# RomanJuranek/librectify

Hardware: AMD Instinct MI355X
Metric: Mpix/s end-to-end (detect+VP) on 4K frames, batch call of 64 frames, 5 in flight (higher is better)
Workload: dtype f32

## Files before the change

librectify_amd/csrc/kernels_fit.hip:

```cpp
#include <algorithm>
#include <cstring>

#include <atomic>

#include "common.h"

namespace lramd {
namespace {

constexpr uint32_t kNoComp = 0xFFFFFFFFu;

constexpr uint32_t kSortLds = 1024;
constexpr uint32_t kSortLdsBig = 16384;
constexpr uint32_t kHugeShift = 14;
constexpr uint32_t kHugeFlag = 0x80000000u;
constexpr int kOffPer = 8;
constexpr uint32_t kOffChunk = 256 * kOffPer;

__device__ __forceinline__ void chunk_counts(const int32_t* __restrict__ seed_size, uint32_t n_seeds, int min_size, int fit_min,
                                             uint32_t k0, int (&sz)[kOffPer], uint32_t& c, uint32_t& p, uint32_t& rc, uint32_t& rp) {
    c = p = rc = rp = 0;
#pragma unroll
    for (int j = 0; j < kOffPer; ++j) {
        sz[j] = (k0 + j < n_seeds) ? seed_size[k0 + j] : 0;
        if (sz[j] > min_size) {
            rc += 1u;
            rp += (uint32_t)sz[j];
        }
        if (sz[j] > fit_min) {
            c += 1u;
            p += (uint32_t)sz[j];
        }
    }
}

__global__ __launch_bounds__(256) void component_offsets_kernel(const int32_t* __restrict__ seed_size,
                                                                const uint32_t* __restrict__ n_ptr, uint32_t cap,
                                                                int min_size, int fit_min, unsigned long long* __restrict__ status, uint32_t tag,
                                                                uint32_t* __restrict__ comp_rank,
                                                                uint32_t* __restrict__ comp_seed,
                                                                uint32_t* __restrict__ comp_off,
                                                                uint32_t* __restrict__ totals, uint32_t* __restrict__ fit_totals,
                                                                uint32_t* __restrict__ large_list,
                                                                uint32_t large_cap, uint32_t* __restrict__ n_large,
                                                                uint32_t* __restrict__ cursor, uint32_t* __restrict__ huge_list,
                                                                uint32_t huge_max) {
    __shared__ uint32_t s_c[4], s_p[4], s_cc[4], s_cp[4], s_rc[4], s_rp[4];
    const uint32_t n_seeds = min(*n_ptr, cap);
    const int tid = threadIdx.x, lane = tid & 63, wv = tid >> 6;
    const uint32_t k0 = blockIdx.x * kOffChunk + (uint32_t)tid * kOffPer;
    int sz[kOffPer];
    uint32_t c, p, rc, rp;
    chunk_counts(seed_size, n_seeds, min_size, fit_min, k0, sz, c, p, rc, rp);
    uint32_t ic = c, ip = p;
#pragma unroll
    for (int off = 1; off < 64; off <<= 1) {
        const uint32_t tc = (uint32_t)__shfl_up((int)ic, off);
        const uint32_t tp = (uint32_t)__shfl_up((int)ip, off);
        if (lane >= off) {
            ic += tc;
            ip += tp;
        }
    }
#pragma unroll
    for (int off = 32; off >= 1; off >>= 1) {
        rc += (uint32_t)__shfl_xor((int)rc, off);
        rp += (uint32_t)__shfl_xor((int)rp, off);
    }
    if (lane == 63) {
        s_c[wv] = ic;
        s_p[wv] = ip;
        s_rc[wv] = rc;
        s_rp[wv] = rp;
    }
    __syncthreads();
    if (tid == 0) {
        const unsigned long long t = (unsigned long long)tag << 32;
        const unsigned long long wc = t | (unsigned long long)(s_c[0] + s_c[1] + s_c[2] + s_c[3]);
        const unsigned long long wp = t | (unsigned long long)(s_p[0] + s_p[1] + s_p[2] + s_p[3]);
        if (blockIdx.x == 0) {
#pragma unroll
            for (int i = 0; i < 4; ++i) __hip_atomic_store(&n_large[i], 0u, __ATOMIC_RELAXED, __HIP_MEMORY_SCOPE_AGENT);
            __hip_atomic_store(&totals[0], 0u, __ATOMIC_RELAXED, __HIP_MEMORY_SCOPE_AGENT);
            __hip_atomic_store(&totals[1], 0u, __ATOMIC_RELAXED, __HIP_MEMORY_SCOPE_AGENT);
            __hip_atomic_store(&status[0], wc, __ATOMIC_RELEASE, __HIP_MEMORY_SCOPE_AGENT);
            __hip_atomic_store(&status[1], wp, __ATOMIC_RELEASE, __HIP_MEMORY_SCOPE_AGENT);
        } else {
            __hip_atomic_store(&status[2u * blockIdx.x], wc, __ATOMIC_RELAXED, __HIP_MEMORY_SCOPE_AGENT);
            __hip_atomic_store(&status[2u * blockIdx.x + 1u], wp, __ATOMIC_RELAXED, __HIP_MEMORY_SCOPE_AGENT);
        }
    }
    uint32_t cc = 0, cp = 0;
    for (uint32_t i = (uint32_t)tid; i < blockIdx.x; i += 256) {
        unsigned long long wc = 0ull, wp = 0ull;
        for (uint32_t spins = 0; spins < (1u << 22); ++spins) {
            wc = __hip_atomic_load(&status[2u * i], __ATOMIC_RELAXED, __HIP_MEMORY_SCOPE_AGENT);
            wp = __hip_atomic_load(&status[2u * i + 1u], __ATOMIC_RELAXED, __HIP_MEMORY_SCOPE_AGENT);
            if ((uint32_t)(wc >> 32) == tag && (uint32_t)(wp >> 32) == tag) break;
            __builtin_amdgcn_s_sleep(2);
        }
        cc += (uint32_t)wc;
        cp += (uint32_t)wp;
    }
#pragma unroll
    for (int off = 32; off >= 1; off >>= 1) {
        cc += (uint32_t)__shfl_xor((int)cc, off);
        cp += (uint32_t)__shfl_xor((int)cp, off);
    }
    if (lane == 0) {
        s_cc[wv] = cc;
        s_cp[wv] = cp;
    }
    __syncthreads();
    if (tid == 0) {
        const uint32_t wrc = s_rc[0] + s_rc[1] + s_rc[2] + s_rc[3], wrp = s_rp[0] + s_rp[1] + s_rp[2] + s_rp[3];
        if (wrc != 0u) {
            __hip_atomic_fetch_add(&totals[0], wrc, __ATOMIC_RELAXED, __HIP_MEMORY_SCOPE_AGENT);
            __hip_atomic_fetch_add(&totals[1], wrp, __ATOMIC_RELAXED, __HIP_MEMORY_SCOPE_AGENT);
        }
    }
    uint32_t rank = s_cc[0] + s_cc[1] + s_cc[2] + s_cc[3] + ic - c;
    uint32_t off_px = s_cp[0] + s_cp[1] + s_cp[2] + s_cp[3] + ip - p;
    for (int i = 0; i < wv; ++i) {
        rank += s_c[i];
        off_px += s_p[i];
    }
#pragma unroll
    for (int j = 0; j < kOffPer; ++j) {
        const uint32_t k = k0 + j;
        if (k < n_seeds) {
            const bool keep = sz[j] > fit_min;
            comp_rank[k] = keep ? rank : kNoComp;
            if (keep) {
                comp_seed[rank] = k;
                comp_off[rank] = off_px;
                if (sz[j] > (int)kSortLds) large_list[large_cap - 1u - atomicAdd(n_large + 1, 1u)] = rank;
                else if (sz[j] > 64) large_list[atomicAdd(n_large, 1u)] = rank;
                uint32_t cur = 0u;
                if (sz[j] > (int)kSortLdsBig && huge_max != 0u) {
                    const uint32_t hi = atomicAdd(n_large + 2, 1u);
                    if (hi < huge_max) {
                        cur = hi | kHugeFlag;
                        huge_list[hi] = rank;
                    }
                }
                cursor[rank] = cur;
                rank += 1u;
                off_px += (uint32_t)sz[j];
            }
        }
    }
    if (blockIdx.x == gridDim.x - 1 && tid == 255) {
        fit_totals[0] = rank;
        fit_totals[1] = off_px;
        comp_off[rank] = off_px;
    }
}

__global__ __launch_bounds__(256) void component_scatter_kernel(const uint32_t* __restrict__ label, size_t npix,
                                                                const uint32_t* __restrict__ comp_rank,
                                                                const uint32_t* __restrict__ comp_off,
                                                                uint32_t* __restrict__ cursor,
                                                                uint32_t* __restrict__ px, uint32_t* __restrict__ huge_tab,
                                                                uint32_t nb) {
    const int lane = threadIdx.x & 63;
    const size_t step = (size_t)gridDim.x * 256;
    const size_t n_pad = (npix + 255) / 256 * 256;
    constexpr int kU = 4;
    for (size_t i0 = (size_t)blockIdx.x * 256 + threadIdx.x; i0 < n_pad; i0 += step * kU) {
        uint32_t l[kU], r[kU];
#pragma unroll
        for (int u = 0; u < kU; ++u) {
            const size_t i = i0 + step * (size_t)u;
            l[u] = i < npix ? label[i] : kLabelFree;
        }
#pragma unroll
        for (int u = 0; u < kU; ++u) r[u] = l[u] != kLabelFree ? comp_rank[l[u]] : kNoComp;
#pragma unroll
        for (int u = 0; u < kU; ++u) {
            const size_t i = i0 + step * (size_t)u;
            if (i >= n_pad) break;
            uint64_t todo = __ballot(r[u] != kNoComp);
            while (todo != 0ull) {
                const int leader = __builtin_ctzll(todo);
                const uint32_t rl = (uint32_t)__builtin_amdgcn_readlane((int)r[u], leader);
                const uint64_t same = __ballot(r[u] == rl) & todo;
                uint32_t base = 0;
                if (lane == leader) {
                    const uint32_t o0 = comp_off[rl], o1 = comp_off[rl + 1u];
                    uint32_t hi = 0u;
                    if (o1 - o0 > kSortLdsBig) hi = cursor[rl];
                    if (hi & kHugeFlag) base = atomicAdd(&huge_tab[(size_t)(hi & ~kHugeFlag) * nb + (uint32_t)(i >> kHugeShift)], (uint32_t)__popcll(same));
                    else base = o0 + atomicAdd(&cursor[rl], (uint32_t)__popcll(same));
                }
                base = (uint32_t)__builtin_amdgcn_readlane((int)base, leader);
                if ((same >> lane) & 1ull) px[base + (uint32_t)__popcll(same & ((1ull << lane) - 1ull))] = (uint32_t)i;
                todo &= ~same;
            }
        }
    }
}

__device__ inline float wave_tree(float v) {
#pragma unroll
    for (int off = 32; off >= 1; off >>= 1) v = v + __shfl_xor(v, off);
    return v;
}

__device__ inline void major_axis_2x2(float a_, float b_, float c_, float& d_r, float& d_c) {
    const double a = a_, b = b_, c = c_;
    const double hd = (a - c) * 0.5;
    const double rad = sqrt(hd * hd + b * b);
    const double lmax = (a + c) * 0.5 + rad;
    double vr, vc;
    if (a >= c) {
        vr = lmax - c;
        vc = b;
    } else {
        vr = b;
        vc = lmax - a;
    }
    const double nn = sqrt(vr * vr + vc * vc);
    if (nn > 0.0) {
        vr = vr / nn;
        vc = vc / nn;
    } else {
        vr = 1.0;
        vc = 0.0;
    }
    float fr = (float)vr, fc = (float)vc;
    if (fr < fc || (fr == fc && fr < 0.0f)) {
        fr = -fr;
        fc = -fc;
    }
    d_r = fr;
    d_c = fc;
}

template <int kThreads, class Keys>
__device__ __forceinline__ void bitonic_sort(Keys& key, uint32_t P) {
    for (uint32_t k = 2; k <= P; k <<= 1)
        for (uint32_t j = k >> 1; j > 0; j >>= 1) {
            for (uint32_t t = threadIdx.x; t < P / 2; t += kThreads) {
                const uint32_t i = 2 * t - (t & (j - 1));
                const uint32_t a = key[i], b = key[i + j];
                const bool up = (i & k) == 0;
                if ((a > b) == up) {
                    key[i] = b;
                    key[i + j] = a;
                }
            }
            __syncthreads();
        }
}

__global__ __launch_bounds__(256) void component_sort_large_kernel(const uint32_t* __restrict__ px_in,
                                                                   uint32_t* __restrict__ px_out,
                                                                   const uint32_t* __restrict__ comp_off,
                                                                   const uint32_t* __restrict__ large_list,
                                                                   const uint32_t* __restrict__ n_large) {
    __shared__ uint32_t s_key[kSortLds];
    const uint32_t n_list = n_large[0];
    for (uint32_t li = blockIdx.x; li < n_list; li += gridDim.x) {
        const uint32_t comp = large_list[li];
        const uint32_t off = comp_off[comp];
        const uint32_t n = comp_off[comp + 1] - off;
        uint32_t P = 128;
        while (P < n) P <<= 1;
        for (uint32_t i = threadIdx.x; i < P; i += 256) s_key[i] = i < n ? px_in[off + i] : 0xFFFFFFFFu;
        __syncthreads();
        bitonic_sort<256>(s_key, P);
        for (uint32_t i = threadIdx.x; i < n; i += 256) px_out[off + i] = s_key[i];
        __syncthreads();
    }
}

template <bool kGlobal>
__global__ __launch_bounds__(1024) void component_sort_big_kernel(const uint32_t* __restrict__ px_in,
                                                                  uint32_t* __restrict__ px_out,
                                                                  const uint32_t* __restrict__ comp_off,
                                                                  const uint32_t* __restrict__ large_list,
                                                                  uint32_t large_cap,
                                                                  const uint32_t* __restrict__ n_large,
                                                                  uint32_t* __restrict__ scratch,
                                                                  const uint32_t* __restrict__ cursor) {
    __shared__ uint32_t s_key[kGlobal ? 1 : kSortLdsBig];
    const uint32_t n_list = n_large[1];
    for (uint32_t li = blockIdx.x; li < n_list; li += gridDim.x) {
        const uint32_t comp = large_list[large_cap - 1u - li];
        const uint32_t off = comp_off[comp];
        const uint32_t n = comp_off[comp + 1] - off;
        if ((n > kSortLdsBig) != kGlobal) continue;
        if (kGlobal && cursor != nullptr && (cursor[comp] & kHugeFlag)) continue;
        uint32_t P = 2048;
        while (P < n) P <<= 1;
        if (!kGlobal) {
            for (uint32_t i = threadIdx.x; i < P; i += 1024) s_key[i] = i < n ? px_in[off + i] : 0xFFFFFFFFu;
            __syncthreads();
            bitonic_sort<1024>(s_key, P);
            for (uint32_t i = threadIdx.x; i < n; i += 1024) px_out[off + i] = s_key[i];
            __syncthreads();
        } else {
            for (uint32_t i = threadIdx.x; i < P; i += 1024) scratch[i] = i < n ? px_in[off + i] : 0xFFFFFFFFu;
            __syncthreads();
            bitonic_sort<1024>(scratch, P);
            for (uint32_t i = threadIdx.x; i < n; i += 1024) px_out[off + i] = scratch[i];
            __syncthreads();
        }
    }
}

__global__ __launch_bounds__(256) void huge_count_kernel(const uint32_t* __restrict__ label, size_t npix,
                                                         const uint32_t* __restrict__ comp_rank,
                                                         const uint32_t* __restrict__ comp_off,
                                                         const uint32_t* __restrict__ cursor, uint32_t* __restrict__ huge_tab,
                                                         uint32_t nb, const uint32_t* __restrict__ huge_list, uint32_t huge_max,
                                                         uint4* __restrict__ jobs, uint32_t* __restrict__ n_large) {
    const uint32_t n_huge = min(n_large[2], huge_max);
    if (n_huge == 0u) return;
    const int lane = threadIdx.x & 63;
    const size_t step = (size_t)gridDim.x * 256;
    const size_t n_pad = (npix + 255) / 256 * 256;
    for (size_t i = (size_t)blockIdx.x * 256 + threadIdx.x; i < n_pad; i += step) {
        const uint32_t l = i < npix ? label[i] : kLabelFree;
        const uint32_t r = l != kLabelFree ? comp_rank[l] : kNoComp;
        uint32_t hi = 0u;
        if (r != kNoComp && comp_off[r + 1u] - comp_off[r] > kSortLdsBig) hi = cursor[r];
        uint64_t todo = __ballot((hi & kHugeFlag) != 0u);
        while (todo != 0ull) {
            const int leader = __builtin_ctzll(todo);
            const uint32_t hl = (uint32_t)__builtin_amdgcn_readlane((int)hi, leader);
            const uint64_t same = __ballot(hi == hl) & todo;
            if (lane == leader) atomicAdd(&huge_tab[(size_t)(hl & ~kHugeFlag) * nb + (uint32_t)(i >> kHugeShift)], (uint32_t)__popcll(same));
            todo &= ~same;
        }
    }
    __shared__ uint32_t s_last;
    __syncthreads();
    if (threadIdx.x == 0) {
        __threadfence();
        s_last = atomicAdd(n_large + 6, 1u) == gridDim.x - 1u ? 1u : 0u;
    }
    __syncthreads();
    if (s_last == 0u) return;
    __threadfence();
    if (threadIdx.x == 0) n_large[6] = 0u;
    for (uint32_t h = threadIdx.x >> 6; h < n_huge; h += 4u) {
        const uint32_t rank = huge_list[h];
        uint32_t run = comp_off[rank];
        for (uint32_t b0 = 0; b0 < nb; b0 += 64u) {
            const uint32_t b = b0 + (uint32_t)lane;
            uint32_t* e = &huge_tab[(size_t)h * nb + b];
            const uint32_t cnt = b < nb ? __hip_atomic_load(e, __ATOMIC_RELAXED, __HIP_MEMORY_SCOPE_AGENT) : 0u;
            uint32_t inc = cnt;
#pragma unroll
            for (int off = 1; off < 64; off <<= 1) {
                const uint32_t t = (uint32_t)__shfl_up((int)inc, off);
                if (lane >= off) inc += t;
            }
            const uint32_t start = run + inc - cnt;
            if (cnt != 0u) {
                *e = start;
                jobs[atomicAdd(n_large + 3, 1u)] = make_uint4(start, cnt, h * nb + b, 0u);
            }
            run += (uint32_t)__shfl((int)inc, 63);
        }
    }
}

__global__ __launch_bounds__(1024) void huge_sort_kernel(const uint32_t* __restrict__ px_in, uint32_t* __restrict__ px_out,
                                                         const uint4* __restrict__ jobs, uint32_t* __restrict__ huge_tab,
                                                         const uint32_t* __restrict__ n_large) {
    __shared__ uint32_t s_key[kSortLdsBig];
    const uint32_t n_jobs = n_large[3];
    for (uint32_t j = blockIdx.x; j < n_jobs; j += gridDim.x) {
        const uint4 job = jobs[j];
        const uint32_t off = job.x, n = job.y;
        uint32_t P = 64;
        while (P < n) P <<= 1;
        for (uint32_t i = threadIdx.x; i < P; i += 1024) s_key[i] = i < n ? px_in[off + i] : 0xFFFFFFFFu;
        __syncthreads();
        bitonic_sort<1024>(s_key, P);
        for (uint32_t i = threadIdx.x; i < n; i += 1024) px_out[off + i] = s_key[i];
        if (threadIdx.x == 0) huge_tab[job.z] = 0u;
        __syncthreads();
    }
}

template <int kU>
__device__ __forceinline__ void fit_large(const uint32_t* __restrict__ px, uint32_t comp, uint32_t off, uint32_t n, float s, float c,
                                          uint32_t uw, const float* __restrict__ dx, const float* __restrict__ dy,
                                          float* __restrict__ scratch_w, LineSegment* __restrict__ out, int lane) {
    float acc = 0.f;
    for (uint32_t i0 = lane; i0 < n; i0 += 64u * kU) {
        uint32_t p[kU];
        float gx[kU], gy[kU];
#pragma unroll
        for (int u = 0; u < kU; ++u) {
            const uint32_t i = i0 + 64u * (uint32_t)u;
            p[u] = i < n ? px[off + i] : 0u;
        }
#pragma unroll
        for (int u = 0; u < kU; ++u) {
            gx[u] = dx[p[u]];
            gy[u] = dy[p[u]];
        }
#pragma unroll
        for (int u = 0; u < kU; ++u) {
            const uint32_t i = i0 + 64u * (uint32_t)u;
            if (i < n) {
                const float wv = directional(gx[u], gy[u], s, c);
                scratch_w[off + i] = wv;
                acc = acc + wv;
            }
        }
    }
    const float S = wave_tree(acc);

    float ar = 0.f, ac = 0.f;
    for (uint32_t i0 = lane; i0 < n; i0 += 64u * kU) {
        uint32_t p[kU];
        float wq[kU];
#pragma unroll
        for (int u = 0; u < kU; ++u) {
            const uint32_t i = i0 + 64u * (uint32_t)u;
            p[u] = i < n ? px[off + i] : 0u;
            wq[u] = i < n ? scratch_w[off + i] : 0.f;
        }
#pragma unroll
        for (int u = 0; u < kU; ++u) {
            const uint32_t i = i0 + 64u * (uint32_t)u;
            if (i < n) {
                const float r = (float)(p[u] / uw), cc = (float)(p[u] % uw);
                const float wn = wq[u] / S;
                ar = ar + wn * r;
                ac = ac + wn * cc;
            }
        }
    }
    const float a_r = wave_tree(ar), a_c = wave_tree(ac);

    float crr = 0.f, crc = 0.f, ccc = 0.f;
    for (uint32_t i0 = lane; i0 < n; i0 += 64u * kU) {
        uint32_t p[kU];
        float wq[kU];
#pragma unroll
        for (int u = 0; u < kU; ++u) {
            const uint32_t i = i0 + 64u * (uint32_t)u;
            p[u] = i < n ? px[off + i] : 0u;
            wq[u] = i < n ? scratch_w[off + i] : 0.f;
        }
#pragma unroll
        for (int u = 0; u < kU; ++u) {
            const uint32_t i = i0 + 64u * (uint32_t)u;
            if (i < n) {
                const float cr = (float)(p[u] / uw) - a_r, cc = (float)(p[u] % uw) - a_c;
                const float wn = wq[u] / S;
                const float t = cr * wn, u2 = cc * wn;
                crr = crr + t * cr;
                crc = crc + t * cc;
                ccc = ccc + u2 * cc;
            }
        }
    }
    const float cov_rr = wave_tree(crr), cov_rc = wave_tree(crc), cov_cc = wave_tree(ccc);

    float d_r, d_c;
    major_axis_2x2(cov_rr, cov_rc, cov_cc, d_r, d_c);
    const float n_r = -d_c, n_c = d_r;

    float t0 = INFINITY, t1 = -INFINITY, es = 0.f;
    for (uint32_t i0 = lane; i0 < n; i0 += 64u * kU) {
        uint32_t p[kU];
#pragma unroll
        for (int u = 0; u < kU; ++u) {
            const uint32_t i = i0 + 64u * (uint32_t)u;
            p[u] = i < n ? px[off + i] : 0u;
        }
#pragma unroll
        for (int u = 0; u < kU; ++u) {
            const uint32_t i = i0 + 64u * (uint32_t)u;
            if (i < n) {
                const float cr = (float)(p[u] / uw) - a_r, cc = (float)(p[u] % uw) - a_c;
                const float t = cr * d_r + cc * d_c;
                t0 = fminf(t0, t);
                t1 = fmaxf(t1, t);
                es = es + fabsf(cr * n_r + cc * n_c);
            }
        }
    }
#pragma unroll
    for (int o = 32; o >= 1; o >>= 1) {
        t0 = fminf(t0, __shfl_xor(t0, o));
        t1 = fmaxf(t1, __shfl_xor(t1, o));
    }
    const float esum = wave_tree(es);
    if (lane == 0) {
        LineSegment l;
        l.x1 = a_c + d_c * t0;
        l.y1 = a_r + d_r * t0;
        l.x2 = a_c + d_c * t1;
        l.y2 = a_r + d_r * t1;
        l.weight = S / (float)n;
        l.err = esum / (float)n;
        l.group_id = -1;
        out[comp] = l;
    }
}

__global__ __launch_bounds__(256) void fit_kernel(const uint32_t* __restrict__ px, const uint32_t* __restrict__ px_unsorted,
                                                  const uint32_t* __restrict__ comp_off,
                                                  const uint32_t* __restrict__ comp_seed, const uint32_t* __restrict__ n_comp_ptr,
                                                  const int32_t* __restrict__ seed_bin, const float* __restrict__ dx,
                                                  const float* __restrict__ dy, int w, BinTrig trig,
                                                  float* __restrict__ scratch_w, LineSegment* __restrict__ out,
                                                  const uint32_t* __restrict__ huge_cursor) {
    const int lane = threadIdx.x & 63;
    const uint32_t comp = blockIdx.x * 4 + (threadIdx.x >> 6);
    if (comp >= *n_comp_ptr) return;
    const uint32_t off = comp_off[comp];
    const uint32_t n = comp_off[comp + 1] - off;
    const int b = seed_bin[comp_seed[comp]];
    const float s = trig.st[b], c = trig.ct[b];
    const uint32_t uw = (uint32_t)w;

    if (n <= 64u) {
        const bool has = (uint32_t)lane < n;
        const uint32_t key = has ? px_unsorted[off + lane] : 0xFFFFFFFFu;
        uint32_t rank = 0;
#pragma unroll
        for (int j = 0; j < 64; ++j) rank += ((uint32_t)__builtin_amdgcn_readlane((int)key, j) < key) ? 1u : 0u;
        const uint32_t p_sorted = (uint32_t)__builtin_amdgcn_ds_permute((int)(min(rank, 63u) << 2), (int)key);
        const uint32_t p = has ? p_sorted : 0u;
        float wv = 0.f;
        if (has) wv = directional(dx[p], dy[p], s, c);
        float acc = 0.f;
        if (has) acc = acc + wv;
        const float S = wave_tree(acc);
        const float r = (float)(p / uw), cq = (float)(p % uw);
        const float wn = wv / S;
        float ar = 0.f, ac = 0.f;
        if (has) {
            ar = ar + wn * r;
            ac = ac + wn * cq;
        }
        const float a_r = wave_tree(ar), a_c = wave_tree(ac);
        const float cr = r - a_r, cc = cq - a_c;
        float crr = 0.f, crc = 0.f, ccc = 0.f;
        if (has) {
            const float t = cr * wn, u = cc * wn;
            crr = crr + t * cr;
            crc = crc + t * cc;
            ccc = ccc + u * cc;
        }
        const float cov_rr = wave_tree(crr), cov_rc = wave_tree(crc), cov_cc = wave_tree(ccc);
        float d_r, d_c;
        major_axis_2x2(cov_rr, cov_rc, cov_cc, d_r, d_c);
        const float n_r = -d_c, n_c = d_r;
        float t0 = INFINITY, t1 = -INFINITY, es = 0.f;
        if (has) {
            const float t = cr * d_r + cc * d_c;
            t0 = fminf(t0, t);
            t1 = fmaxf(t1, t);
            es = es + fabsf(cr * n_r + cc * n_c);
        }
#pragma unroll
        for (int o = 32; o >= 1; o >>= 1) {
            t0 = fminf(t0, __shfl_xor(t0, o));
            t1 = fmaxf(t1, __shfl_xor(t1, o));
        }
        const float esum = wave_tree(es);
        if (lane == 0) {
            LineSegment l;
            l.x1 = a_c + d_c * t0;
            l.y1 = a_r + d_r * t0;
            l.x2 = a_c + d_c * t1;
            l.y2 = a_r + d_r * t1;
            l.weight = S / (float)n;
            l.err = esum / (float)n;
            l.group_id = -1;
            out[comp] = l;
        }
        return;
    }

    if (huge_cursor != nullptr && n > kSortLdsBig && (huge_cursor[comp] & kHugeFlag) != 0u) return;
    fit_large<8>(px, comp, off, n, s, c, uw, dx, dy, scratch_w, out, lane);
}

__device__ __forceinline__ float huge_chunk_sum(float acc, const float* __restrict__ v, uint32_t cn, int lane) {
    for (uint32_t j0 = (uint32_t)lane; j0 < cn; j0 += 64u * 16u) {
        float t[16];
#pragma unroll
        for (int u = 0; u < 16; ++u) {
            const uint32_t j = j0 + 64u * (uint32_t)u;
            t[u] = j < cn ? v[j] : 0.f;
        }
#pragma unroll
        for (int u = 0; u < 16; ++u)
            if (j0 + 64u * (uint32_t)u < cn) acc = acc + t[u];
    }
    return acc;
}
constexpr int kHugeTerms = 24576;
constexpr size_t kHugeLdsBytes = (size_t)kHugeTerms * sizeof(float);
__global__ __launch_bounds__(1024) void fit_huge_kernel(const uint32_t* __restrict__ px, const uint32_t* __restrict__ comp_off,
                                                        const uint32_t* __restrict__ comp_seed, const uint32_t* __restrict__ huge_list,
                                                        const uint32_t* __restrict__ n_large, uint32_t huge_max,
                                                        const int32_t* __restrict__ seed_bin, const float* __restrict__ dx,
                                                        const float* __restrict__ dy, int w, BinTrig trig,
                                                        float* __restrict__ scratch_w, LineSegment* __restrict__ out) {
    extern __shared__ float s_terms[];
    __shared__ float s_res[3];
    __shared__ float s_mm[2][16];
    if (blockIdx.x >= min(n_large[2], huge_max)) return;
    const uint32_t comp = huge_list[blockIdx.x];
    const uint32_t off = comp_off[comp];
    const uint32_t n = comp_off[comp + 1] - off;
    const int b = seed_bin[comp_seed[comp]];
    const float s = trig.st[b], c = trig.ct[b];
    const uint32_t uw = (uint32_t)w;
    const int tid = (int)threadIdx.x, lane = tid & 63, wave = tid >> 6;

    float acc = 0.f;
    {
        constexpr uint32_t kC = 16384u;
        constexpr int kE = (int)(kC / 1024u);
        for (uint32_t c0 = 0; c0 < n; c0 += kC) {
            const uint32_t cn = min(kC, n - c0);
            uint32_t p[kE];
            float gx[kE], gy[kE];
#pragma unroll
            for (int e = 0; e < kE; ++e) {
                const uint32_t j = (uint32_t)tid + 1024u * (uint32_t)e;
                p[e] = j < cn ? px[off + c0 + j] : 0u;
            }
#pragma unroll
            for (int e = 0; e < kE; ++e) {
                gx[e] = dx[p[e]];
                gy[e] = dy[p[e]];
            }
#pragma unroll
            for (int e = 0; e < kE; ++e) {
                const uint32_t j = (uint32_t)tid + 1024u * (uint32_t)e;
                if (j < cn) {
                    const float wv = directional(gx[e], gy[e], s, c);
                    scratch_w[off + c0 + j] = wv;
                    s_terms[j] = wv;
                }
            }
            __syncthreads();
            if (wave == 0) acc = huge_chunk_sum(acc, s_terms, cn, lane);
            __syncthreads();
        }
    }
    if (wave == 0) {
        const float t = wave_tree(acc);
        if (lane == 0) s_res[0] = t;
    }
    __syncthreads();
    const float S = s_res[0];
    __syncthreads();

    acc = 0.f;
    {
        constexpr uint32_t kC = kHugeTerms / 2;
        constexpr int kE = (int)(kC / 1024u);
        for (uint32_t c0 = 0; c0 < n; c0 += kC) {
            const uint32_t cn = min(kC, n - c0);
            uint32_t q[kE];
            float wq[kE];
#pragma unroll
            for (int e = 0; e < kE; ++e) {
                const uint32_t j = (uint32_t)tid + 1024u * (uint32_t)e;
                q[e] = j < cn ? px[off + c0 + j] : 0u;
                wq[e] = j < cn ? scratch_w[off + c0 + j] : 0.f;
            }
#pragma unroll
            for (int e = 0; e < kE; ++e) {
                const uint32_t j = (uint32_t)tid + 1024u * (uint32_t)e;
                if (j < cn) {
                    const float r = (float)(q[e] / uw), cc = (float)(q[e] % uw);
                    const float wn = wq[e] / S;
                    s_terms[j] = wn * r;
                    s_terms[kC + j] = wn * cc;
                }
            }
            __syncthreads();
            if (wave < 2) acc = huge_chunk_sum(acc, s_terms + (size_t)wave * kC, cn, lane);
            __syncthreads();
        }
    }
    if (wave < 2) {
        const float t = wave_tree(acc);
        if (lane == 0) s_res[wave] = t;
    }
    __syncthreads();
    const float a_r = s_res[0], a_c = s_res[1];
    __syncthreads();

    acc = 0.f;
    {
        constexpr uint32_t kC = kHugeTerms / 3;
        constexpr int kE = (int)(kC / 1024u);
        static_assert(kC % 1024u == 0u, "a chunk is a whole number of elements per thread");
        for (uint32_t c0 = 0; c0 < n; c0 += kC) {
            const uint32_t cn = min(kC, n - c0);
            uint32_t q[kE];
            float wq[kE];
#pragma unroll
            for (int e = 0; e < kE; ++e) {
                const uint32_t j = (uint32_t)tid + 1024u * (uint32_t)e;
                q[e] = j < cn ? px[off + c0 + j] : 0u;
                wq[e] = j < cn ? scratch_w[off + c0 + j] : 0.f;
            }
#pragma unroll
            for (int e = 0; e < kE; ++e) {
                const uint32_t j = (uint32_t)tid + 1024u * (uint32_t)e;
                if (j < cn) {
                    const float cr = (float)(q[e] / uw) - a_r, cc = (float)(q[e] % uw) - a_c;
                    const float wn = wq[e] / S;
                    const float t = cr * wn, u2 = cc * wn;
                    s_terms[j] = t * cr;
                    s_terms[kC + j] = t * cc;
                    s_terms[2u * kC + j] = u2 * cc;
                }
            }
            __syncthreads();
            if (wave < 3) acc = huge_chunk_sum(acc, s_terms + (size_t)wave * kC, cn, lane);
            __syncthreads();
        }
    }
    if (wave < 3) {
        const float t = wave_tree(acc);
        if (lane == 0) s_res[wave] = t;
    }
    __syncthreads();
    const float cov_rr = s_res[0], cov_rc = s_res[1], cov_cc = s_res[2];
    __syncthreads();

    float d_r, d_c;
    major_axis_2x2(cov_rr, cov_rc, cov_cc, d_r, d_c);
    const float n_r = -d_c, n_c = d_r;

    float t0 = INFINITY, t1 = -INFINITY;
    acc = 0.f;
    {
        constexpr uint32_t kC = kHugeTerms;
        constexpr int kE = (int)(kC / 1024u);
        for (uint32_t c0 = 0; c0 < n; c0 += kC) {
            const uint32_t cn = min(kC, n - c0);
            uint32_t q[kE];
#pragma unroll
            for (int e = 0; e < kE; ++e) {
                const uint32_t j = (uint32_t)tid + 1024u * (uint32_t)e;
                q[e] = j < cn ? px[off + c0 + j] : 0u;
            }
#pragma unroll
            for (int e = 0; e < kE; ++e) {
                const uint32_t j = (uint32_t)tid + 1024u * (uint32_t)e;
                if (j < cn) {
                    const float cr = (float)(q[e] / uw) - a_r, cc = (float)(q[e] % uw) - a_c;
                    const float t = cr * d_r + cc * d_c;
                    t0 = fminf(t0, t);
                    t1 = fmaxf(t1, t);
                    s_terms[j] = fabsf(cr * n_r + cc * n_c);
                }
            }
            __syncthreads();
            if (wave == 0) acc = huge_chunk_sum(acc, s_terms, cn, lane);
            __syncthreads();
        }
    }
#pragma unroll
    for (int o = 32; o >= 1; o >>= 1) {
        t0 = fminf(t0, __shfl_xor(t0, o));
        t1 = fmaxf(t1, __shfl_xor(t1, o));
    }
    if (lane == 0) {
        s_mm[0][wave] = t0;
        s_mm[1][wave] = t1;
    }
    __syncthreads();
    if (wave != 0) return;
    const float esum = wave_tree(acc);
    if (lane == 0) {
        for (int i = 1; i < 16; ++i) {
            t0 = fminf(t0, s_mm[0][i]);
            t1 = fmaxf(t1, s_mm[1][i]);
        }
        LineSegment l;
        l.x1 = a_c + d_c * t0;
        l.y1 = a_r + d_r * t0;
        l.x2 = a_c + d_c * t1;
        l.y2 = a_r + d_r * t1;
        l.weight = S / (float)n;
        l.err = esum / (float)n;
        l.group_id = -1;
        out[comp] = l;
    }
}

}

size_t fit_temp_bytes(size_t max_pixels, uint32_t max_segments) {
    (void)max_segments;
    return (max_pixels / kOffChunk + 2) * 2 * sizeof(unsigned long long) + 256;
}

int launch_component_offsets(const int32_t* seed_size, const uint32_t* d_n_seeds, uint32_t seed_cap, int min_size, int fit_min,
                             uint32_t* comp_rank, uint32_t* comp_seed, uint32_t* comp_off, uint32_t* totals, uint32_t* fit_totals,
                             uint32_t* large_list, uint32_t large_cap, uint32_t* n_large, void* temp, size_t temp_bytes,
                             uint32_t frame_tag, uint32_t* cursor, const HugeSort& hs, hipStream_t s) {
    const uint32_t chunks = (seed_cap + kOffChunk - 1) / kOffChunk;
    if (chunks == 0 || temp_bytes < (size_t)chunks * 2 * sizeof(unsigned long long)) {
        set_error("launch_component_offsets: workspace too small");
        return 1;
    }
    if (fit_min < min_size) {
        set_error("launch_component_offsets: fit threshold below the size threshold");
        return 1;
    }
    hipLaunchKernelGGL(component_offsets_kernel, dim3(chunks), dim3(256), 0, s, seed_size, d_n_seeds, seed_cap, min_size, fit_min,
                       static_cast<unsigned long long*>(temp), frame_tag, comp_rank, comp_seed, comp_off, totals, fit_totals, large_list, large_cap,
                       n_large, cursor, hs.list, hs.tab ? hs.max : 0u);
    LR_HIP(hipGetLastError());
    return 0;
}

int launch_component_scatter(const uint32_t* label, size_t npix, const uint32_t* comp_rank, const uint32_t* comp_off,
                             uint32_t* cursor, uint32_t* px, const HugeSort& hs, uint32_t* n_large, bool with_huge, hipStream_t s) {
    const uint32_t nb = (uint32_t)((npix + ((size_t)1 << kHugeShift) - 1) >> kHugeShift);
    const size_t want = (npix + 255) / 256;
    if (with_huge && hs.tab)
        hipLaunchKernelGGL(huge_count_kernel, dim3((unsigned)std::min<size_t>(want, 2048)), dim3(256), 0, s, label, npix, comp_rank, comp_off,
                           cursor, hs.tab, nb, hs.list, hs.max, reinterpret_cast<uint4*>(hs.jobs), n_large);
    const int blocks = (int)(want < 8192 ? want : 8192);
    hipLaunchKernelGGL(component_scatter_kernel, dim3(blocks > 0 ? blocks : 1), dim3(256), 0, s, label, npix, comp_rank,
                       comp_off, cursor, px, hs.tab, nb);
    LR_HIP(hipGetLastError());
    return 0;
}

int launch_component_sort(const uint32_t* px_in, uint32_t* px_out, const uint32_t* comp_off, const uint32_t* d_n_comp,
                          uint32_t comp_cap, const uint32_t* large_list, uint32_t large_cap, const uint32_t* n_large,
                          uint32_t* scratch, const uint32_t* cursor, const HugeSort& hs, bool with_huge, hipStream_t s) {
    if (comp_cap == 0) return 0;
    (void)d_n_comp;
    hipLaunchKernelGGL(component_sort_large_kernel, dim3(4096), dim3(256), 0, s, px_in, px_out, comp_off, large_list, n_large);
    hipLaunchKernelGGL(component_sort_big_kernel<false>, dim3(128), dim3(1024), 0, s, px_in, px_out, comp_off, large_list,
                       large_cap, n_large, scratch, cursor);
    if (with_huge && hs.tab) {
        hipLaunchKernelGGL(huge_sort_kernel, dim3(512), dim3(1024), 0, s, px_in, px_out, reinterpret_cast<const uint4*>(hs.jobs), hs.tab, n_large);
        hipLaunchKernelGGL(component_sort_big_kernel<true>, dim3(1), dim3(1024), 0, s, px_in, px_out, comp_off, large_list,
                           large_cap, n_large, scratch, cursor);
    }
    LR_HIP(hipGetLastError());
    return 0;
}

int launch_fit(const uint32_t* px_sorted, const uint32_t* px_unsorted, const uint32_t* comp_off, const uint32_t* comp_seed, const uint32_t* d_n_comp,
               uint32_t comp_cap, const int32_t* seed_bin, const float* dx, const float* dy, int w, BinTrig trig,
               float* scratch_w, LineSegment* out, const uint32_t* cursor, const HugeSort& hs, const uint32_t* n_large, bool with_huge,
               hipStream_t s) {
    if (comp_cap == 0) return 0;
    const bool huge = with_huge && hs.tab != nullptr && hs.max != 0u;
    if (huge) {
        static std::atomic<uint64_t> done_mask{0};
        int dev = 0;
        LR_HIP(hipGetDevice(&dev));
        const uint64_t bit = 1ull << (dev & 63);
        if (!(done_mask.load(std::memory_order_acquire) & bit)) {
            LR_HIP(hipFuncSetAttribute(reinterpret_cast<const void*>(fit_huge_kernel), hipFuncAttributeMaxDynamicSharedMemorySize, (int)kHugeLdsBytes));
            done_mask.fetch_or(bit, std::memory_order_release);
        }
        hipLaunchKernelGGL(fit_huge_kernel, dim3(hs.max), dim3(1024), kHugeLdsBytes, s, px_sorted, comp_off, comp_seed, hs.list, n_large, hs.max, seed_bin,
                           dx, dy, w, trig, scratch_w, out);
    }
    hipLaunchKernelGGL(fit_kernel, dim3((comp_cap + 3) / 4), dim3(256), 0, s, px_sorted, px_unsorted, comp_off, comp_seed, d_n_comp,
                       seed_bin, dx, dy, w, trig, scratch_w, out, huge ? cursor : nullptr);
    LR_HIP(hipGetLastError());
    return 0;
}

}
```

librectify_amd/csrc/kernels_seeds.hip:

```cpp
#include <algorithm>
#include <cstdlib>
#include <cstring>

#include "common.h"

namespace lramd {
namespace {

__global__ __launch_bounds__(256) void seed_count_kernel(const uint64_t* __restrict__ cand,
                                                         const uint32_t* __restrict__ cand_count,
                                                         const uint32_t* __restrict__ tile_max, int n_tiles, int cand_cap,
                                                         float keep_ratio, float* __restrict__ maxmag,
                                                         uint32_t* __restrict__ tile_pass) {
    __shared__ uint32_t s_red[4];
    const int lane = threadIdx.x & 63, wave = threadIdx.x >> 6;
    uint32_t m = 0;
    for (int i0 = threadIdx.x; i0 < n_tiles; i0 += 256 * 8) {
        uint32_t v[8];
#pragma unroll
        for (int k = 0; k < 8; ++k) {
            const int i = i0 + k * 256;
            v[k] = i < n_tiles ? tile_max[i] : 0u;
        }
#pragma unroll
        for (int k = 0; k < 8; ++k) m = max(m, v[k]);
    }
#pragma unroll
    for (int off = 32; off >= 1; off >>= 1) m = max(m, (uint32_t)__shfl_xor((int)m, off));
    if (lane == 0) s_red[wave] = m;
    __syncthreads();
    const float mx = __uint_as_float(max(max(s_red[0], s_red[1]), max(s_red[2], s_red[3])));
    if (blockIdx.x == 0 && threadIdx.x == 0) *maxmag = mx;
    const float thr = mx * keep_ratio;
    const int tile = blockIdx.x * 4 + wave;
    if (tile >= n_tiles) return;
    const uint32_t n = cand_count[tile];
    const uint64_t* c = cand + (size_t)tile * cand_cap;
    uint32_t cnt = 0;
    for (uint32_t i = lane; i < n; i += 64) cnt += (__uint_as_float((uint32_t)(c[i] >> 32)) > thr) ? 1u : 0u;
#pragma unroll
    for (int off = 32; off >= 1; off >>= 1) cnt += (uint32_t)__shfl_xor((int)cnt, off);
    if (lane == 0) tile_pass[tile] = cnt;
}

__global__ __launch_bounds__(1024) void seed_scan_kernel(const uint32_t* __restrict__ tile_pass, int n_tiles,
                                                         uint32_t* __restrict__ tile_off, uint32_t* __restrict__ n_seeds) {
    __shared__ uint32_t s_wave[16];
    const int lane = threadIdx.x & 63, wave = threadIdx.x >> 6;
    const int K = (n_tiles + 1023) / 1024;
    const int i0 = (int)threadIdx.x * K, i1 = min(n_tiles, i0 + K);
    uint32_t sum = 0;
    for (int b0 = i0; b0 < i1; b0 += 8) {
        uint32_t v[8];
#pragma unroll
        for (int k = 0; k < 8; ++k) v[k] = b0 + k < i1 ? tile_pass[b0 + k] : 0u;
#pragma unroll
        for (int k = 0; k < 8; ++k) sum += v[k];
    }
    uint32_t inc = sum;
#pragma unroll
    for (int off = 1; off < 64; off <<= 1) {
        const uint32_t o = (uint32_t)__shfl_up((int)inc, off);
        if (lane >= off) inc += o;
    }
    if (lane == 63) s_wave[wave] = inc;
    __syncthreads();
    uint32_t before = 0, total = 0;
#pragma unroll
    for (int w2 = 0; w2 < 16; ++w2) {
        const uint32_t t = s_wave[w2];
        before += w2 < wave ? t : 0u;
        total += t;
    }
    uint32_t run = before + inc - sum;
    for (int b0 = i0; b0 < i1; b0 += 8) {
        uint32_t v[8];
#pragma unroll
        for (int k = 0; k < 8; ++k) v[k] = b0 + k < i1 ? tile_pass[b0 + k] : 0u;
#pragma unroll
        for (int k = 0; k < 8; ++k)
            if (b0 + k < i1) {
                tile_off[b0 + k] = run;
                run += v[k];
            }
    }
    if (threadIdx.x == 0) *n_seeds = total;
}

__global__ __launch_bounds__(256) void seed_write_kernel(const uint64_t* __restrict__ cand,
                                                         const uint32_t* __restrict__ cand_count, int n_tiles,
                                                         int cand_cap, const float* __restrict__ maxmag,
                                                         float keep_ratio, const uint32_t* __restrict__ tile_pass,
                                                         const uint32_t* __restrict__ tile_off,
                                                         uint64_t* __restrict__ keys, uint32_t cap) {
    const int tile = blockIdx.x * 4 + (threadIdx.x >> 6);
    const int lane = threadIdx.x & 63;
    if (tile >= n_tiles) return;
    const float thr = *maxmag * keep_ratio;
    const uint32_t n = cand_count[tile];
    const uint64_t* c = cand + (size_t)tile * cand_cap;
    uint32_t base = tile_off[tile];
    for (uint32_t i0 = 0; i0 < n; i0 += 64) {
        const uint32_t i = i0 + lane;
        uint64_t k = 0;
        bool pass = false;
        if (i < n) {
            k = c[i];
            pass = __uint_as_float((uint32_t)(k >> 32)) > thr;
        }
        const uint64_t m = __ballot(pass);
        if (pass) {
            const uint32_t pos = base + (uint32_t)__popcll(m & ((1ull << lane) - 1ull));
            if (pos < cap) keys[pos] = ((uint64_t)(~(uint32_t)(k >> 32)) << 32) | (k & 0xFFFFFFFFull);
        }
        base += (uint32_t)__popcll(m);
    }
}

constexpr int kSelBands = 2048;
__global__ __launch_bounds__(256) void seed_select_kernel(const uint64_t* __restrict__ cand, const uint32_t* __restrict__ cand_count,
                                                          const uint32_t* __restrict__ tile_max, int n_tiles, int cand_cap, int per_wg,
                                                          float keep_ratio, float* __restrict__ maxmag,
                                                          unsigned long long* __restrict__ status, uint32_t tag,
                                                          uint64_t* __restrict__ keys, uint32_t cap, uint32_t* __restrict__ n_seeds) {
    __shared__ uint32_t s_red[4], s_sum[4];
    __shared__ uint32_t s_cnt[kSelBands];
    __shared__ uint32_t s_total;
    const int lane = threadIdx.x & 63, wave = threadIdx.x >> 6;
    uint32_t m = 0;
    for (int i0 = threadIdx.x; i0 < n_tiles; i0 += 256 * 8) {
        uint32_t v[8];
#pragma unroll
        for (int k = 0; k < 8; ++k) {
            const int i = i0 + k * 256;
            v[k] = i < n_tiles ? tile_max[i] : 0u;
        }
#pragma unroll
        for (int k = 0; k < 8; ++k) m = max(m, v[k]);
    }
#pragma unroll
    for (int off = 32; off >= 1; off >>= 1) m = max(m, (uint32_t)__shfl_xor((int)m, off));
    if (lane == 0) s_red[wave] = m;
    __syncthreads();
    const float mx = __uint_as_float(max(max(s_red[0], s_red[1]), max(s_red[2], s_red[3])));
    if (blockIdx.x == 0 && threadIdx.x == 0) *maxmag = mx;
    const float thr = mx * keep_ratio;
    const int t0 = (int)blockIdx.x * per_wg, t1 = min(n_tiles, t0 + per_wg);
    for (int t = t0 + wave; t < t1; t += 4) {
        const uint32_t n = cand_count[t];
        const uint64_t* c = cand + (size_t)t * cand_cap;
        uint32_t cnt = 0;
        for (uint32_t i = lane; i < n; i += 64) cnt += (__uint_as_float((uint32_t)(c[i] >> 32)) > thr) ? 1u : 0u;
#pragma unroll
        for (int off = 32; off >= 1; off >>= 1) cnt += (uint32_t)__shfl_xor((int)cnt, off);
        if (lane == 0) s_cnt[t - t0] = cnt;
    }
    __syncthreads();
    const int nb = max(t1 - t0, 0);
    if (wave == 0) {
        uint32_t run = 0;
        for (int c0 = 0; c0 < nb; c0 += 64) {
            const uint32_t v = c0 + lane < nb ? s_cnt[c0 + lane] : 0u;
            uint32_t inc = v;
#pragma unroll
            for (int off = 1; off < 64; off <<= 1) {
                const uint32_t o = (uint32_t)__shfl_up((int)inc, off);
                if (lane >= off) inc += o;
            }
            if (c0 + lane < nb) s_cnt[c0 + lane] = run + inc - v;
            run += (uint32_t)__shfl((int)inc, 63);
        }
        if (lane == 0) {
            s_total = run;
            __hip_atomic_store(&status[blockIdx.x], ((unsigned long long)tag << 32) | (unsigned long long)run, __ATOMIC_RELAXED,
                               __HIP_MEMORY_SCOPE_AGENT);
        }
    }
    uint32_t before = 0;
    for (uint32_t j = threadIdx.x; j < blockIdx.x; j += 256) {
        unsigned long long w = 0ull;
        for (uint32_t spins = 0; spins < (1u << 22); ++spins) {
            w = __hip_atomic_load(&status[j], __ATOMIC_RELAXED, __HIP_MEMORY_SCOPE_AGENT);
            if ((uint32_t)(w >> 32) == tag) break;
            __builtin_amdgcn_s_sleep(2);
        }
        before += (uint32_t)w;
    }
#pragma unroll
    for (int off = 32; off >= 1; off >>= 1) before += (uint32_t)__shfl_xor((int)before, off);
    if (lane == 0) s_sum[wave] = before;
    __syncthreads();
    const uint32_t base0 = s_sum[0] + s_sum[1] + s_sum[2] + s_sum[3];
    if (blockIdx.x == gridDim.x - 1 && threadIdx.x == 0) *n_seeds = base0 + s_total;
    for (int t = t0 + wave; t < t1; t += 4) {
        const uint32_t n = cand_count[t];
        const uint64_t* c = cand + (size_t)t * cand_cap;
        uint32_t base = base0 + s_cnt[t - t0];
        for (uint32_t i0 = 0; i0 < n; i0 += 64) {
            const uint32_t i = i0 + lane;
            uint64_t k = 0;
            bool pass = false;
            if (i < n) {
                k = c[i];
                pass = __uint_as_float((uint32_t)(k >> 32)) > thr;
            }
            const uint64_t mm = __ballot(pass);
            if (pass) {
                const uint32_t pos = base + (uint32_t)__popcll(mm & ((1ull << lane) - 1ull));
                if (pos < cap) keys[pos] = ((uint64_t)(~(uint32_t)(k >> 32)) << 32) | (k & 0xFFFFFFFFull);
            }
            base += (uint32_t)__popcll(mm);
        }
    }
}

constexpr uint32_t kRun0 = 2048;
constexpr uint32_t kRunThreads = kRun0 / 4;
constexpr uint32_t kFinalRuns = 16;

__device__ __forceinline__ uint64_t shfl_xor_u64(uint64_t v, int lane_mask) {
    const uint32_t lo = (uint32_t)__shfl_xor((int)(uint32_t)v, lane_mask);
    const uint32_t hi = (uint32_t)__shfl_xor((int)(uint32_t)(v >> 32), lane_mask);
    return ((uint64_t)hi << 32) | lo;
}
__global__ __launch_bounds__(kRunThreads) void seed_run_sort_kernel(uint64_t* __restrict__ keys, uint32_t cap,
                                                            const uint32_t* __restrict__ n_ptr) {
    __shared__ uint64_t sk[kRun0];
    const uint32_t n = min(*n_ptr, cap);
    const uint32_t base = blockIdx.x * kRun0;
    if (base >= n) return;
    const uint32_t t = threadIdx.x, i0 = 4u * t;
    uint64_t e[4];
#pragma unroll
    for (int r = 0; r < 4; ++r) e[r] = (base + i0 + r < n) ? keys[base + i0 + r] : ~0ull;
#define LR_KEEP(own, other, i, j, k) ((((((i) & (j)) == 0u) == (((i) & (k)) == 0u)) == ((other) < (own))) ? (other) : (own))
    for (uint32_t k = 2; k <= kRun0; k <<= 1) {
        for (uint32_t j = k >> 1; j > 0; j >>= 1) {
            if (j >= 256u) {
#pragma unroll
                for (int r = 0; r < 4; ++r) sk[i0 + r] = e[r];
                __syncthreads();
                uint64_t o[4];
#pragma unroll
                for (int r = 0; r < 4; ++r) o[r] = sk[(i0 + r) ^ j];
                __syncthreads();
#pragma unroll
                for (int r = 0; r < 4; ++r) e[r] = LR_KEEP(e[r], o[r], i0 + r, j, k);
            } else if (j >= 4u) {
                const int lm = (int)(j >> 2);
#pragma unroll
                for (int r = 0; r < 4; ++r) {
                    const uint64_t o = shfl_xor_u64(e[r], lm);
                    e[r] = LR_KEEP(e[r], o, i0 + r, j, k);
                }
            } else {
                const bool two = j == 2u;
                const uint64_t o0 = two ? e[2] : e[1], o1 = two ? e[3] : e[0], o2 = two ? e[0] : e[3], o3 = two ? e[1] : e[2];
                e[0] = LR_KEEP(e[0], o0, i0 + 0u, j, k);
                e[1] = LR_KEEP(e[1], o1, i0 + 1u, j, k);
                e[2] = LR_KEEP(e[2], o2, i0 + 2u, j, k);
                e[3] = LR_KEEP(e[3], o3, i0 + 3u, j, k);
            }
        }
    }
#undef LR_KEEP
#pragma unroll
    for (int r = 0; r < 4; ++r)
        if (base + i0 + r < n) keys[base + i0 + r] = e[r];
}

__device__ __forceinline__ uint32_t count_below(const uint64_t* __restrict__ run, uint32_t L, uint32_t valid, uint64_t key) {
    uint32_t lo = 0;
    for (uint32_t sstep = L >> 1; sstep > 0; sstep >>= 1) {
        const uint32_t pos = lo + sstep - 1u;
        const uint64_t v = pos < valid ? run[pos] : ~0ull;
        lo += v < key ? sstep : 0u;
    }
    return lo + ((lo == L - 1u && L - 1u < valid && run[L - 1u] < key) ? 1u : 0u);
}

__global__ __launch_bounds__(256) void seed_merge_kernel(const uint64_t* __restrict__ in, uint64_t* __restrict__ out, uint32_t L,
                                                         uint32_t cap, const uint32_t* __restrict__ n_ptr) {
    const uint32_t g = blockIdx.x * 256 + threadIdx.x;
    const uint32_t n = min(*n_ptr, cap);
    if (g >= n) return;
    const uint32_t r = g / L, i = g - r * L, q = r ^ 1u;
    const uint64_t key = in[g];
    const uint32_t qbase = q * L;
    const uint32_t valid = qbase < n ? min(L, n - qbase) : 0u;
    const uint32_t below = valid ? count_below(in + qbase, L, valid, key) : 0u;
    out[(size_t)(r & ~1u) * L + i + below] = key;
}

__global__ __launch_bounds__(256) void seed_rank_setup_kernel(const uint64_t* __restrict__ keys, const uint32_t* __restrict__ n_ptr,
                                                              uint32_t cap, uint32_t L, const float* __restrict__ dx,
                                                              const float* __restrict__ dy, BinTrig trig, float trace_tolerance,
                                                              int32_t* __restrict__ seed_idx, int32_t* __restrict__ seed_bin,
                                                              float* __restrict__ seed_thr, uint4* __restrict__ seed_rec) {
    const uint32_t g = blockIdx.x * 256 + threadIdx.x;
    const uint32_t n = min(*n_ptr, cap);
    if (g >= n) return;
    const uint32_t n_runs = (n + L - 1u) / L;
    const uint32_t mine = g / L;
    const uint64_t key = keys[g];
    uint32_t rank = g - mine * L;
    for (uint32_t q0 = 0; q0 < n_runs; q0 += 8u) {
        uint32_t lo[8], valid[8];
#pragma unroll
        for (int j = 0; j < 8; ++j) {
            const uint32_t q = q0 + (uint32_t)j;
            lo[j] = 0u;
            valid[j] = (q < n_runs && q != mine) ? min(L, n - q * L) : 0u;
        }
        for (uint32_t sstep = L >> 1; sstep > 0; sstep >>= 1) {
            uint64_t v[8];
#pragma unroll
            for (int j = 0; j < 8; ++j) {
                const uint32_t pos = lo[j] + sstep - 1u;
                v[j] = pos < valid[j] ? keys[(size_t)(q0 + (uint32_t)j) * L + pos] : ~0ull;
            }
#pragma unroll
            for (int j = 0; j < 8; ++j) lo[j] += v[j] < key ? sstep : 0u;
        }
#pragma unroll
        for (int j = 0; j < 8; ++j) {
            if (lo[j] == L - 1u && L - 1u < valid[j] && keys[(size_t)(q0 + (uint32_t)j) * L + L - 1u] < key) lo[j] += 1u;
            rank += lo[j];
        }
    }
    const uint32_t low = (uint32_t)key;
    const uint32_t idx = low >> 3;
    const int bin = (int)(low & 7u);
    const float v = directional(dx[idx], dy[idx], trig.st[bin], trig.ct[bin]);
    seed_idx[rank] = (int32_t)idx;
    seed_bin[rank] = bin;
    const float thr = (1 - trace_tolerance) * v;
    seed_thr[rank] = thr;
    seed_rec[rank] = make_uint4(idx, (uint32_t)bin, __float_as_uint(thr), 0u);
}

}

int launch_seed_order(uint64_t* keys, uint64_t* keys_alt, const uint32_t* n_seeds, uint32_t cap, const float* dx, const float* dy,
                      BinTrig trig, float trace_tolerance, int32_t* seed_idx, int32_t* seed_bin, float* seed_thr, uint4* seed_rec, hipStream_t s) {
    if (cap == 0) return 0;
    const uint32_t runs0 = (cap + kRun0 - 1) / kRun0;
    hipLaunchKernelGGL(seed_run_sort_kernel, dim3(runs0), dim3(kRunThreads), 0, s, keys, cap, n_seeds);
    uint32_t L = kRun0, runs = runs0;
    uint64_t* cur = keys;
    uint64_t* nxt = keys_alt;
    while (runs > 1u && (runs > kFinalRuns || (uint64_t)cap * runs > ((uint64_t)4 << 20))) {
        hipLaunchKernelGGL(seed_merge_kernel, dim3((cap + 255) / 256), dim3(256), 0, s, cur, nxt, L, cap, n_seeds);
        std::swap(cur, nxt);
        L *= 2u;
        runs = (runs + 1u) / 2u;
    }
    hipLaunchKernelGGL(seed_rank_setup_kernel, dim3((cap + 255) / 256), dim3(256), 0, s, cur, n_seeds, cap, L, dx, dy, trig,
                       trace_tolerance, seed_idx, seed_bin, seed_thr, seed_rec);
    LR_HIP(hipGetLastError());
    return 0;
}

size_t seeds_temp_bytes(int n_tiles, size_t max_seeds) {
    (void)n_tiles;
    (void)max_seeds;
    return 256;
}

int launch_seed_select(const uint64_t* cand, const uint32_t* cand_count, const uint32_t* tile_max, int n_tiles,
                       int cand_cap, float seed_keep_ratio, float* maxmag, uint32_t* tile_pass, uint32_t* tile_off, uint64_t* keys,
                       uint32_t key_cap, uint32_t* n_seeds, uint32_t frame_tag, hipStream_t s) {
    static const bool fused = !(std::getenv("LIBRECTIFY_SEED_SELECT_FUSED") && std::atoi(std::getenv("LIBRECTIFY_SEED_SELECT_FUSED")) == 0);
    if (fused && frame_tag != 0u && n_tiles > 0) {
        int wgs = std::min(256, (n_tiles + 3) / 4);
        int per_wg = (n_tiles + wgs - 1) / wgs;
        if (per_wg > kSelBands) {
            per_wg = kSelBands;
            wgs = (n_tiles + per_wg - 1) / per_wg;
        }
        wgs = (n_tiles + per_wg - 1) / per_wg;
        hipLaunchKernelGGL(seed_select_kernel, dim3(wgs), dim3(256), 0, s, cand, cand_count, tile_max, n_tiles, cand_cap, per_wg,
                           seed_keep_ratio, maxmag, reinterpret_cast<unsigned long long*>(tile_off), frame_tag, keys, key_cap, n_seeds);
        LR_HIP(hipGetLastError());
        return 0;
    }
    const int blocks = (n_tiles + 3) / 4;
    hipLaunchKernelGGL(seed_count_kernel, dim3(blocks), dim3(256), 0, s, cand, cand_count, tile_max, n_tiles, cand_cap,
                       seed_keep_ratio, maxmag, tile_pass);
    hipLaunchKernelGGL(seed_scan_kernel, dim3(1), dim3(1024), 0, s, tile_pass, n_tiles, tile_off, n_seeds);
    hipLaunchKernelGGL(seed_write_kernel, dim3(blocks), dim3(256), 0, s, cand, cand_count, n_tiles, cand_cap, maxmag,
                       seed_keep_ratio, tile_pass, tile_off, keys, key_cap);
    LR_HIP(hipGetLastError());
    return 0;
}

}
```

Before: 10750.

## Sort per-component pixel lists with register-resident bitonic network and wave shuffles

Replaces the shared-memory bitonic sort used for large and big connected components with a sort that keeps 4–16 keys per thread in registers. Early stages run inside each thread, mid-distance stages use cross-lane shuffles, and only long-distance stages go through LDS. The goal is to cut the many LDS round trips and block-wide barriers of the old per-step LDS bitonic network. A shared sort_network.h header is added, and the LDS buffer for the list kernel grows to 4096 words. The larger buffer and higher register use may lower occupancy.

```diff
diff --git a/librectify_amd/csrc/kernels_fit.hip b/librectify_amd/csrc/kernels_fit.hip
--- a/librectify_amd/csrc/kernels_fit.hip
+++ b/librectify_amd/csrc/kernels_fit.hip
@@ -4,13 +4,14 @@
 #include <atomic>
 
 #include "common.h"
+#include "sort_network.h"
 
 namespace lramd {
 namespace {
 
 constexpr uint32_t kNoComp = 0xFFFFFFFFu;
 
-constexpr uint32_t kSortLds = 1024;
+constexpr uint32_t kSortLds = 4096;
 constexpr uint32_t kSortLdsBig = 16384;
 constexpr uint32_t kHugeShift = 14;
 constexpr uint32_t kHugeFlag = 0x80000000u;
@@ -237,6 +238,84 @@
     d_c = fc;
 }
 
+template <int kThreads, int K>
+__device__ __forceinline__ void sort_list_in_registers(const uint32_t* __restrict__ in, uint32_t* __restrict__ out, uint32_t n,
+                                                       uint32_t P, uint32_t* __restrict__ s_key) {
+    const uint32_t t = threadIdx.x, i0 = (uint32_t)K * t;
+    const uint32_t n_active = sort_active_threads(P, K);
+    const bool active = t < n_active;
+    uint32_t e[K];
+#pragma unroll
+    for (int r = 0; r < K; ++r) {
+        const uint32_t i = sort_load_index(t, (uint32_t)r, n_active);
+        e[r] = (active && i < n) ? in[i] : kSortPad;
+    }
+    if (active) sort_first_stages<K>(e, i0);
+    for (uint32_t k = 2u * K; k <= P; k <<= 1) {
+        for (uint32_t j = k >> 1; j >= (uint32_t)K; j >>= 1) {
+            if (sort_pass_in_lds(j, K, 64u)) {
+                const uint32_t tp = t ^ (j / (uint32_t)K);
+                if (active) {
+#pragma unroll
+                    for (int r = 0; r < K; ++r) s_key[sort_lds_word(t, (uint32_t)r, kThreads)] = e[r];
+                }
+                __syncthreads();
+                uint32_t o[K];
+                if (active) {
+#pragma unroll
+                    for (int r = 0; r < K; ++r) o[r] = s_key[sort_lds_word(tp, (uint32_t)r, kThreads)];
+                }
+                __syncthreads();
+                if (active) sort_keep<K>(e, o, i0, j, k);
+            } else if (active) {
+                const int lm = (int)(j / (uint32_t)K);
+                uint32_t o[K];
+#pragma unroll
+                for (int r = 0; r < K; ++r) o[r] = (uint32_t)__shfl_xor((int)e[r], lm);
+                sort_keep<K>(e, o, i0, j, k);
+            }
+        }
+        if (active) sort_in_thread<K>(e, i0, k);
+    }
+#pragma unroll
+    for (int r = 0; r < K; ++r)
+        if (i0 + (uint32_t)r < n) out[i0 + (uint32_t)r] = e[r];
+}
+
+__global__ __launch_bounds__(256) void component_sort_list_kernel(const uint32_t* __restrict__ px_in, uint32_t* __restrict__ px_out,
+                                                                  const uint32_t* __restrict__ comp_off,
+                                                                  const uint32_t* __restrict__ large_list,
+                                                                  const uint32_t* __restrict__ n_large) {
+    __shared__ uint32_t s_key[kSortLds];
+    const uint32_t n_list = n_large[0];
+    for (uint32_t li = blockIdx.x; li < n_list; li += gridDim.x) {
+        const uint32_t comp = large_list[li];
+        const uint32_t off = comp_off[comp];
+        const uint32_t n = comp_off[comp + 1] - off;
+        const uint32_t P = sort_padded(n);
+        switch (sort_keys_per_thread(P, 256u)) {
+            case 4u: sort_list_in_registers<256, 4>(px_in + off, px_out + off, n, P, s_key); break;
+            case 8u: sort_list_in_registers<256, 8>(px_in + off, px_out + off, n, P, s_key); break;
+            default: sort_list_in_registers<256, 16>(px_in + off, px_out + off, n, P, s_key); break;
+        }
+    }
+}
+
+__global__ __launch_bounds__(1024) void component_sort_long_kernel(const uint32_t* __restrict__ px_in, uint32_t* __restrict__ px_out,
+                                                                   const uint32_t* __restrict__ comp_off,
+                                                                   const uint32_t* __restrict__ large_list, uint32_t large_cap,
+                                                                   const uint32_t* __restrict__ n_large) {
+    __shared__ uint32_t s_key[kSortLdsBig];
+    const uint32_t n_list = n_large[1];
+    for (uint32_t li = blockIdx.x; li < n_list; li += gridDim.x) {
+        const uint32_t comp = large_list[large_cap - 1u - li];
+        const uint32_t off = comp_off[comp];
+        const uint32_t n = comp_off[comp + 1] - off;
+        if (n > kSortLdsBig) continue;
+        sort_list_in_registers<1024, 16>(px_in + off, px_out + off, n, sort_padded(n), s_key);
+    }
+}
+
 template <int kThreads, class Keys>
 __device__ __forceinline__ void bitonic_sort(Keys& key, uint32_t P) {
     for (uint32_t k = 2; k <= P; k <<= 1)
@@ -252,27 +331,6 @@
             }
             __syncthreads();
         }
-}
-
-__global__ __launch_bounds__(256) void component_sort_large_kernel(const uint32_t* __restrict__ px_in,
-                                                                   uint32_t* __restrict__ px_out,
-                                                                   const uint32_t* __restrict__ comp_off,
-                                                                   const uint32_t* __restrict__ large_list,
-                                                                   const uint32_t* __restrict__ n_large) {
-    __shared__ uint32_t s_key[kSortLds];
-    const uint32_t n_list = n_large[0];
-    for (uint32_t li = blockIdx.x; li < n_list; li += gridDim.x) {
-        const uint32_t comp = large_list[li];
-        const uint32_t off = comp_off[comp];
-        const uint32_t n = comp_off[comp + 1] - off;
-        uint32_t P = 128;
-        while (P < n) P <<= 1;
-        for (uint32_t i = threadIdx.x; i < P; i += 256) s_key[i] = i < n ? px_in[off + i] : 0xFFFFFFFFu;
-        __syncthreads();
-        bitonic_sort<256>(s_key, P);
-        for (uint32_t i = threadIdx.x; i < n; i += 256) px_out[off + i] = s_key[i];
-        __syncthreads();
-    }
 }
 
 template <bool kGlobal>
@@ -847,9 +905,9 @@
                           uint32_t* scratch, const uint32_t* cursor, const HugeSort& hs, bool with_huge, hipStream_t s) {
     if (comp_cap == 0) return 0;
     (void)d_n_comp;
-    hipLaunchKernelGGL(component_sort_large_kernel, dim3(4096), dim3(256), 0, s, px_in, px_out, comp_off, large_list, n_large);
-    hipLaunchKernelGGL(component_sort_big_kernel<false>, dim3(128), dim3(1024), 0, s, px_in, px_out, comp_off, large_list,
-                       large_cap, n_large, scratch, cursor);
+    hipLaunchKernelGGL(component_sort_list_kernel, dim3(4096), dim3(256), 0, s, px_in, px_out, comp_off, large_list, n_large);
+    hipLaunchKernelGGL(component_sort_long_kernel, dim3(128), dim3(1024), 0, s, px_in, px_out, comp_off, large_list, large_cap,
+                       n_large);
     if (with_huge && hs.tab) {
         hipLaunchKernelGGL(huge_sort_kernel, dim3(512), dim3(1024), 0, s, px_in, px_out, reinterpret_cast<const uint4*>(hs.jobs), hs.tab, n_large);
         hipLaunchKernelGGL(component_sort_big_kernel<true>, dim3(1), dim3(1024), 0, s, px_in, px_out, comp_off, large_list,
diff --git a/librectify_amd/csrc/kernels_seeds.hip b/librectify_amd/csrc/kernels_seeds.hip
--- a/librectify_amd/csrc/kernels_seeds.hip
+++ b/librectify_amd/csrc/kernels_seeds.hip
@@ -3,6 +3,7 @@
 #include <cstring>
 
 #include "common.h"
+#include "sort_network.h"
 
 namespace lramd {
 namespace {
@@ -233,7 +234,6 @@
     uint64_t e[4];
 #pragma unroll
     for (int r = 0; r < 4; ++r) e[r] = (base + i0 + r < n) ? keys[base + i0 + r] : ~0ull;
-#define LR_KEEP(own, other, i, j, k) ((((((i) & (j)) == 0u) == (((i) & (k)) == 0u)) == ((other) < (own))) ? (other) : (own))
     for (uint32_t k = 2; k <= kRun0; k <<= 1) {
         for (uint32_t j = k >> 1; j > 0; j >>= 1) {
             if (j >= 256u) {
@@ -263,7 +263,6 @@
             }
         }
     }
-#undef LR_KEEP
 #pragma unroll
     for (int r = 0; r < 4; ++r)
         if (base + i0 + r < n) keys[base + i0 + r] = e[r];
diff --git a/librectify_amd/csrc/sort_network.h b/librectify_amd/csrc/sort_network.h
--- /dev/null
+++ b/librectify_amd/csrc/sort_network.h
@@ -0,0 +1,55 @@
+#pragma once
+#include <cstdint>
+
+#if defined(__HIPCC__) || defined(__CUDACC__)
+#define LR_SORT_HD __host__ __device__ __forceinline__
+#define LR_SORT_UNROLL _Pragma("unroll")
+#else
+#define LR_SORT_HD inline
+#define LR_SORT_UNROLL
+#endif
+
+#define LR_KEEP(own, other, i, j, k) ((((((i) & (j)) == 0u) == (((i) & (k)) == 0u)) == ((other) < (own))) ? (other) : (own))
+
+namespace lramd {
+
+constexpr uint32_t kSortPad = 0xFFFFFFFFu;
+constexpr uint32_t kSortMinP = 128;
+
+LR_SORT_HD uint32_t sort_padded(uint32_t n) {
+    uint32_t P = kSortMinP;
+    while (P < n) P <<= 1;
+    return P;
+}
+LR_SORT_HD uint32_t sort_keys_per_thread(uint32_t P, uint32_t threads) { return P <= 4u * threads ? 4u : P <= 8u * threads ? 8u : 16u; }
+LR_SORT_HD uint32_t sort_active_threads(uint32_t P, uint32_t K) { return P / K; }
+LR_SORT_HD uint32_t sort_load_index(uint32_t t, uint32_t r, uint32_t active) { return r * active + t; }
+LR_SORT_HD bool sort_pass_in_lds(uint32_t j, uint32_t K, uint32_t lanes) { return j >= lanes * K; }
+LR_SORT_HD uint32_t sort_lds_word(uint32_t t, uint32_t r, uint32_t threads) { return r * threads + t; }
+
+template <int K>
+LR_SORT_HD void sort_keep(uint32_t (&e)[K], const uint32_t (&o)[K], uint32_t i0, uint32_t j, uint32_t k) {
+    LR_SORT_UNROLL
+    for (int r = 0; r < K; ++r) e[r] = LR_KEEP(e[r], o[r], i0 + (uint32_t)r, j, k);
+}
+template <int K>
+LR_SORT_HD void sort_in_thread_pass(uint32_t (&e)[K], uint32_t i0, int j, uint32_t k) {
+    uint32_t o[K];
+    LR_SORT_UNROLL
+    for (int r = 0; r < K; ++r) o[r] = e[r ^ j];
+    sort_keep<K>(e, o, i0, (uint32_t)j, k);
+}
+template <int K>
+LR_SORT_HD void sort_in_thread(uint32_t (&e)[K], uint32_t i0, uint32_t k) {
+    LR_SORT_UNROLL
+    for (int j = K >> 1; j > 0; j >>= 1) sort_in_thread_pass<K>(e, i0, j, k);
+}
+template <int K>
+LR_SORT_HD void sort_first_stages(uint32_t (&e)[K], uint32_t i0) {
+    LR_SORT_UNROLL
+    for (int k = 2; k <= K; k <<= 1)
+        LR_SORT_UNROLL
+        for (int j = k >> 1; j > 0; j >>= 1) sort_in_thread_pass<K>(e, i0, j, (uint32_t)k);
+}
+
+}
```

After: 10880, median of 3. +1.3%, better.
